# mike-gimelfarb/bboptpy

Hardware: AMD Instinct MI355X
Metric: candidate-evals/sec (higher is better)
Workload: dtype f64; 1 GPU; ActiveCMAES n=128 np=4096 rosenbrock, 256 independent populations per GPU in lockstep; populations_per_gpu=256, n=128, np=4096, objective=rosenbrock

## Files before the change

bboptpy_amd/csrc/bbo_cma.hip:

```cpp
#include "bbo_cma_kernels.hpp"
#include "bbo_sep_kernels.hpp"
#include "bbo_chol_kernels.hpp"
#include "bbo_eig_mw.hpp"

#include <algorithm>
#include <atomic>
#include <cmath>
#include <cstdlib>
#include <limits>

namespace bbo {

namespace {

enum { K_SAMPLE = 0, K_RANK, K_WHITEN, K_GRAM, K_PATHS, K_COV, K_EIGEN, K_POST, K_STOP, K_COUNT };
static const char *const K_NAMES[K_COUNT] = { "bbo:cma_sample_eval", "bbo:cma_rank", "bbo:cma_whiten", "bbo:cma_gram", "bbo:cma_paths", "bbo:cma_cov", "bbo:cma_eigen", "bbo:cma_post", "bbo:cma_history_stop" };

int pick_maxt(int ld)
{
    const int per_wave = ((ld >> 4) + 3) / 4;
    if (per_wave <= 1) return 1;
    if (per_wave <= 2) return 2;
    if (per_wave <= 4) return 4;
    return 8;
// ... 231 lines not shown
        if (params_.adjustlr) c.ccov *= ((n + 2.) / 3.);
    }

    c.rps = 64;
    while (c.rps > 16 && gram_lds_bytes(c.ld, c.rps) > GRAM_LDS_MAX) c.rps >>= 1;
    if (c.ld == 128) {
        int cap = 32;
        if (const char *e = std::getenv("BBO_GRAM_WANT")) cap = std::max(1, std::atoi(e));
        int want = std::max(1, std::min(cap, (512 + P - 1) / P));
        want = std::min(want, (c.lambda_pad + G128_CH - 1) / G128_CH);
        c.rps = ((c.lambda_pad + want - 1) / want + G128_CH - 1) / G128_CH * G128_CH;
    }
    c.splits = (c.lambda_pad + c.rps - 1) / c.rps;
    if (chol) c.splits = 1;
    else if (sep)
        c.splits = std::max(1, std::min(c.mu / 16, (1024 + P - 1) / P));

    const size_t ld = c.ld, ld2 = ld * ld;
    const bool same_shape = dense && keep_bc_ && last_n_ == n && C_.count == P * ld2;
    X_.alloc((size_t) P * c.lambda_pad * ld);
    f_.alloc((size_t) P * c.lambda_pad);
    zn2_.alloc((size_t) P * c.lambda_pad);
    rank_.alloc((size_t) P * c.lambda_pad);
    order_.alloc((size_t) P * c.lambda_pad);
    xmean_.alloc(P * ld);
    xold_.alloc(P * ld);
    pc_.alloc(P * ld);
    ps_.alloc(P * ld);
    D_.alloc(P * ld);
    csep_.alloc(P * ld);
    if (dense) {
        isc_.alloc(P * ld2);
        BDp_.alloc(P * ld2);
        ISp_.alloc(P * ld2);
    }
    if (chol) {
        A_.alloc(P * ld2);
        C_.alloc(P * ld2);
        BDp_.alloc(P * ld2);
        std::vector<double> eyeA(P * ld2, 0.), eyeP(P * ld2, 0.);
        for (int p = 0; p < P; p++)
            for (size_t i = 0; i < (size_t) n; i++) {
                eyeA[p * ld2 + i * ld + i] = 1.;
                eyeP[p * ld2 + bfrag_index(i, i, ld)] = 1.;
            }
        A_.upload(eyeA.data(), P * ld2);
        allow_lds((const void*) chol_factor, 136 * 1024);
        std::vector<int> zero(P, 0);
        chol_repairs_.alloc(P);
        chol_repairs_.upload(zero.data(), P);
        BDp_.upload(eyeP.data(), P * ld2);
    }
    S_.alloc((size_t) P * c.mu_pad);
    gram_part_.alloc((size_t) P * c.splits * (dense ? ld2 : ld));
    mean_part_.alloc((size_t) P * c.splits * ld);
    hist_best_.alloc((size_t) P * c.hlen);
    hist_kth_.alloc((size_t) P * c.hlen);
    weights_.alloc(c.mu);
    weights_.upload(w.data(), c.mu);
    scal_.alloc(P);
    zinject_.release();
    zrecord_.release();
    upload_box(n, c.ld, lower, upper, obj);

    std::vector<double> eye(dense ? P * ld2 : 0, 0.), ones(P * ld, 1.);
    csep_.upload(ones.data(), P * ld);
    if (dense) {
        for (int p = 0; p < P; p++)
            for (int i = 0; i < n; i++) eye[p * ld2 + (size_t) i * ld + i] = 1.;
        if (same_shape) {
            std::vector<double> bm(P * ld2), cm(P * ld2);
            B_.download(bm.data(), P * ld2);
            C_.download(cm.data(), P * ld2);
            for (int p = 0; p < P; p++)
                for (int i = 0; i < n; i++) {
                    bm[p * ld2 + (size_t) i * ld + i] = 1.;
                    cm[p * ld2 + (size_t) i * ld + i] = 1.;
                }
            B_.upload(bm.data(), P * ld2);
            C_.upload(cm.data(), P * ld2);
        } else {
            B_.alloc(P * ld2);
            C_.alloc(P * ld2);
            B_.upload(eye.data(), P * ld2);
            C_.upload(eye.data(), P * ld2);
        }
        isc_.upload(eye.data(), P * ld2);
    }
    D_.upload(ones.data(), P * ld);
    keep_bc_ = dense;
    last_n_ = n;

    std::vector<double> xm(P * ld, 0.);
    for (int p = 0; p < P; p++) std::copy(guess + (size_t) p * n, guess + (size_t) (p + 1) * n,
            xm.begin() + p * ld);
    xmean_.upload(xm.data(), P * ld);

    std::vector<CmaScal> sc(P);
    for (auto &s : sc) {
        std::memset(&s, 0, sizeof(s));
        s.sigma = params_.sigma0;
        s.fbest = -std::numeric_limits<double>::infinity();
        s.fworst = std::numeric_limits<double>::infinity();
        s.hist_head = -1;
        s.basis_ok = same_shape ? 0 : 1;
    }
    scal_.upload(sc.data(), P);
    basis_maybe_stale_ = same_shape;

    if (dense) eig_work_.alloc((size_t) P * 4 * eig_slab((int) ld));

    CmaDev &d = d_;
    d = CmaDev {};
    d.X = X_.p; d.f = f_.p; d.rank = rank_.p; d.order = order_.p;
    d.xmean = xmean_.p; d.xold = xold_.p; d.pc = pc_.p; d.ps = ps_.p;
    d.C = C_.p; d.B = B_.p; d.D = D_.p; d.isc = isc_.p; d.BDp = BDp_.p; d.ISp = ISp_.p;
    d.A = chol ? A_.p : nullptr;
    d.chol_repairs = chol ? chol_repairs_.p : nullptr;
    d.S = S_.p; d.zn2 = zn2_.p; d.csep = csep_.p; d.gram_part = gram_part_.p; d.mean_part = mean_part_.p;
    d.hist_best = hist_best_.p; d.hist_kth = hist_kth_.p; d.eig_work = eig_work_.p;
    d.weights = weights_.p; d.lower = lower_.p; d.upper = upper_.p; d.aux = aux_.p;
    d.zinject = nullptr; d.zrecord = nullptr; d.scal = scal_.p;
    d.stamps = stamps_.p;
    d.mw_fail_host = mw_fail_host_;
    d.mw_fault = mw_fault_from_env();
    mw_release();

    if (obj_.is_program()) {
        prog_.bind(obj_.program, params_.device, n, P);
        std::vector<ProgPlan> plan(P);
        for (int p = 0; p < P; p++)
            plan[p] = ProgPlan { X_.p + (size_t) p * c.lambda_pad * ld, f_.p + (size_t) p * c.lambda_pad, lambda,
                    c.ld };
        prog_.upload_plan(plan);
        std::vector<double> finf((size_t) P * c.lambda_pad, std::numeric_limits<double>::infinity());
        f_.upload(finf.data(), finf.size());
    } else
        prog_.unbind();

    c.honor_stop = 0;
    inited_ = true;
    if (dense) {
        launch_post(2);
        BBO_HIP(hipGetLastError());
        BBO_HIP(hipStreamSynchronize(stream_));
    }
}

void CmaEngine::launch_post(int mode)
{
    const CmaConst &c = c_;
    if (c.ld <= 128) {
        const size_t lds = (size_t) (c.ld * (c.ld + 2) + c.ld) * sizeof(double);
        allow_lds((const void*) cma_post_mfma<1>, 140 * 1024);
        allow_lds((const void*) cma_post_mfma<4>, 140 * 1024);
        if (c.npop < 32)
            hipLaunchKernelGGL(cma_post_mfma<4>, dim3(c.npop, 4), dim3(256), lds, stream_, d_, c_,
                    mode);
        else
            hipLaunchKernelGGL(cma_post_mfma<1>, dim3(c.npop, 1), dim3(256), lds, stream_, d_, c_,
                    mode);
    } else {
        dim3 grid(c.ld / 16, c.ld / 16, c.npop);
        hipLaunchKernelGGL(cma_post, grid, dim3(256), 0, stream_, d_, c_, mode);
    }
}

SampleRoute CmaEngine::sample_route() const
{
    const CmaConst &c = c_;
    SampleRoute r {};
// ... 433 lines not shown
            gens, ldy, scratch);
    BBO_HIP(hipGetLastError());
}

void CmaEngine::generation(bool honor_stop)
{
    if (small_fused_ok()) {
        launch_small(1, honor_stop);
        return;
    }
    small_fused_ = false;
    c_.honor_stop = honor_stop ? 1 : 0;
    launch_sample_eval();
    if (obj_.needs_host()) host_evaluate();
    else if (obj_.is_program()) program_evaluate();
    launch_rank();
    const EigRoute route = eig_route(true, true);
    launch_update(!route.forms_c);
    launch_eigen(route);
    launch_history_stop();
}

void CmaEngine::phase(int which)
{
    BBO_REQUIRE(inited_, "phase before init");
    BBO_HIP(hipSetDevice(params_.device));
    c_.honor_stop = 0;
    d_.mw_fault = mw_fault_from_env();
    switch (which) {
    case BBO_PHASE_SAMPLE_EVALUATE:
        launch_sample_eval();
        if (obj_.needs_host()) host_evaluate();
        else if (obj_.is_program()) program_evaluate();
        break;
    case BBO_PHASE_RANK: launch_rank(); break;
    case BBO_PHASE_UPDATE: launch_update(); break;
    case BBO_PHASE_EIGEN: launch_eigen(eig_route()); break;
    case BBO_PHASE_HISTORY_STOP: launch_history_stop(); break;
    default: throw Error(BBO_ERR_ARG, "unknown CMA phase");
    }
    BBO_HIP(hipStreamSynchronize(stream_));
    if (mw_check_failed() && which == BBO_PHASE_EIGEN) {
        launch_eigen(eig_route());
        BBO_HIP(hipStreamSynchronize(stream_));
    }
    timer_.collect();
    prog_timer_.collect();
}

void CmaEngine::inject_normals(const double *z, int count)
{
    BBO_REQUIRE(inited_, "inject_normals before init");
    rank_wrote_norms_ = false;
    if (!z) {
        d_.zinject = nullptr;
        return;
    }
    const size_t want = (size_t) c_.npop * c_.lambda * c_.n;
    BBO_REQUIRE((size_t) count == want, "inject_normals: count must be populations*lambda*n");
    if (zinject_.count != want) zinject_.alloc(want);
    zinject_.upload(z, want);
    d_.zinject = zinject_.p;
}

void CmaEngine::after_chunk(bool in_run)
{
    if (in_run) return;
    if (mw_check_failed()) {
        launch_eigen(eig_route());
        BBO_HIP(hipStreamSynchronize(stream_));
    }
}

void CmaEngine::inspect(const std::vector<CmaScal> &sc)
{
    bool stale = false;
    for (const auto &s : sc) stale = stale || !s.basis_ok;
    basis_maybe_stale_ = stale;
    mw_check_failed();
    for (const auto &s : sc)
        if (s.eig_mw_fail && !mw_disabled_) {
            mw_disabled_ = true;
            mw_release();
        }
}

int CmaEngine::chunk_limit(int want)
{
    return small_fused_ok() ? std::min(want, 512) : want;
}

void CmaEngine::launch_chunk(int gens)
{
    if (small_fused_ok()) launch_small(gens, true);
    else Engine::launch_chunk(gens);
}

void CmaEngine::solution(int population, double *x_out, int *n_evals, int *converged)
{
    enter_population("solution()", population);
    CmaScal s;
    scal_.download(&s, 1, population);
    std::vector<double> x(c_.ld);
    if (s.it <= 0) xmean_.download(x.data(), c_.ld, (size_t) population * c_.ld);
    else X_.download(x.data(), c_.ld, ((size_t) population * c_.lambda_pad + s.ibw[0]) * c_.ld);
    std::copy(x.begin(), x.begin() + c_.n, x_out);
    *n_evals = s.fev;
    if (s.it <= 0) {
        *converged = c_.variant == 3 ? (c_.tol >= 0. ? 1 : 0) : (0 >= c_.mit) ? 1 : 0;
    } else {
        *converged = s.flag != 0 ? 1 : 0;
    }
}

void CmaEngine::optimize(int n, const double *lower, const double *upper, const double *guess,
// ... 121 lines not shown
            for (int i = 0; i < 48; i++) out[i] = (double) t[i];
        }
        return 48;
    }
    if (k == "best_hist" || k == "kth_hist") {
        if (out && cap >= c.hlen)
            (k == "best_hist" ? hist_best_ : hist_kth_).download(out, c.hlen, (size_t) p * c.hlen);
        return c.hlen;
    }
    CmaScal s;
    scal_.download(&s, 1, p);
    if (k == "sigma") return o.one(s.sigma);
    if (k == "it") return o.one(s.it);
    if (k == "fev") return o.one(s.fev);
    if (k == "flag") return o.one(s.flag);
    if (k == "stop") return o.one(s.stop);
    if (k == "hsig") return o.one(s.hsig);
    if (k == "pslen") return o.one(s.pslen);
    if (k == "fbest") return o.one(s.fbest);
    if (k == "fworst") return o.one(s.fworst);
    if (k == "eigenlastev") return o.one(s.eigenlastev);
    if (k == "eigen_done") return o.one(s.eigen_done);
    if (k == "basis_ok") return o.one(s.basis_ok);
    if (k == "eig_stage") return o.one(s.eig_stage);
    if (k == "eig_mw_fail") return o.one(s.eig_mw_fail);
    if (k == "chol_repairs") {
        if (c.variant != 3) throw Error(BBO_ERR_KEY, "'chol_repairs' belongs to CholeskyCMAES");
        int r = 0;
        chol_repairs_.download(&r, 1, p);
        return o.one(r);
    }
    if (c.variant == 3 && k == "chol_tri") return o.one(chol_tri_ ? 1 : 0);
    if (c.variant == 3 && k == "stol") return o.one(c.stol);
    if (c.variant == 3 && k == "ranked") return o.one(c.ranked);
    if (k == "eig_mw_off") return o.one(mw_disabled_ ? 1 : 0);
    if (k == "eig_split_maxp") return o.one(split_maxp_);
    if (k == "eig_fixed128") return o.one(last_route_.fixed ? 1 : 0);
    if (k == "cov_fused") return o.one(last_route_.forms_c ? 1 : 0);
    if (k == "eig_route") {
        double ids[sizeof(last_route_.step) / sizeof(last_route_.step[0])];
        for (int i = 0; i < last_route_.count; i++) ids[i] = last_route_.step[i].k;
        return o.copy(ids, last_route_.count);
    }
    if (k == "rank_route") return o.one(last_rank_);
    if (k == "sample_route") return o.one(last_sample_.k);
    if (k == "sample_lean") return o.one(last_sample_.full);
    if (k == "update_route") {
        double ids[sizeof(last_update_.step) / sizeof(last_update_.step[0])];
        for (int i = 0; i < last_update_.count; i++) ids[i] = last_update_.step[i].k;
        return o.copy(ids, last_update_.count);
    }
    if (k == "small_fused") return o.one(small_fused_ ? 1 : 0);
    if (k == "splits") return o.one(c.splits);
    if (k == "eig_mw_reserved") return o.one((double) mw_reserved_);
    if (k == "eig_mw_capacity") {
        MwBudget &b = MwBudget::get();
        std::lock_guard<std::mutex> lock(b.m);
        return o.one((double) b.capacity(params_.device));
    }
    if (k == "best_len") return o.one(s.hist_len);
    if (k == "best_buffer") return o.one(s.hist_head);
    if (k == "ibest") return o.one(s.ibw[0]);
    if (k == "ybw") return o.copy(s.ybw, 4);
    if (k == "ibw") {
        const double ids[4] = { (double) s.ibw[0], (double) s.ibw[1], (double) s.ibw[2], (double) s.ibw[3] };
        return o.copy(ids, 4);
    }
    if (k == "n") return o.one(c.n);
    if (k == "lambda") return o.one(c.lambda);
    if (k == "mu") return o.one(c.mu);
    if (k == "mueff") return o.one(c.mueff);
    if (k == "cc") return o.one(c.cc);
    if (k == "cs") return o.one(c.cs);
    if (k == "c1") return o.one(c.c1);
    if (k == "cmu") return o.one(c.cmu);
    if (k == "cneg") return o.one(c.cneg);
    if (k == "alphaold") return o.one(c.alphaold);
    if (k == "cm") return o.one(c.cm);
    if (k == "ccov") return o.one(c.ccov);
    if (k == "damps") return o.one(c.damps);
    if (k == "chi") return o.one(c.chi);
    if (k == "eigenfreq") return o.one(c.eigenfreq);
    if (k == "hlen") return o.one(c.hlen);
    if (k == "ik") return o.one(c.ik);
    if (k == "mit") return o.one(c.mit);
    if (k == "mfev") return o.one(c.mfev);
    if (k == "sigma0") return o.one(c.sigma0);
    throw Error(BBO_ERR_KEY, "unknown state key '" + k + "'");
}

int CmaEngine::set(const std::string &k, int p, const double *in, int count)
{
    enter_population("set()", p);
    rank_wrote_norms_ = false;
    const CmaConst &c = c_;
    const size_t ld = c.ld, n = c.n;
    auto vec_in = [&](DevBuf<double> &b) {
        BBO_REQUIRE(count == (int) n, "set: wrong element count");
        upload_rows(b, p, 1, c.n, c.ld, in);
        return count;
    };
    auto mat_in = [&](DevBuf<double> &b) {
        BBO_REQUIRE(count == (int) (n * n), "set: wrong element count");
        std::vector<double> tmp(ld * ld, 0.);
        for (size_t i = 0; i < n; i++) std::copy(in + i * n, in + (i + 1) * n, tmp.begin() + i * ld);
        b.upload(tmp.data(), ld * ld, p * ld * ld);
        return count;
    };
    if (c.variant == 2 && (k == "B" || k == "C" || k == "D"))
        throw Error(BBO_ERR_KEY, "SepCMAES: set 'csep' (D is its square root)");
    if (c.variant == 3 && (k == "B" || k == "C" || k == "D" || k == "csep"))
        throw Error(BBO_ERR_KEY, "CholeskyCMAES keeps the factor: set 'A'");
    if (k == "A") {
        if (c.variant != 3) throw Error(BBO_ERR_KEY, "'A' belongs to CholeskyCMAES");
        BBO_REQUIRE(count == (int) (n * n), "set: wrong element count");
        std::vector<double> a(ld * ld, 0.), pk(ld * ld, 0.);
        for (size_t i = 0; i < n; i++)
            for (size_t j = 0; j <= i; j++) {
                a[i * ld + j] = in[i * n + j];
                pk[bfrag_index(i, j, ld)] = in[i * n + j];
            }
        A_.upload(a.data(), ld * ld, p * ld * ld);
        BDp_.upload(pk.data(), ld * ld, p * ld * ld);
        return count;
    }
    if (c.variant == 3 && k == "arx") {
        BBO_REQUIRE(count == (int) (c.lambda * n), "set: wrong element count");
        upload_rows(X_, (size_t) p * c.lambda_pad, c.lambda, c.n, c.ld, in);
        return count;
    }
    if (k == "fitness") {
        BBO_REQUIRE(count == c.lambda, "set: wrong element count");
        std::vector<double> f(in, in + c.lambda);
        nan_to_inf(f.data(), c.lambda);
        f_.upload(f.data(), c.lambda, (size_t) p * c.lambda_pad);
        return count;
    }
    if (k == "xmean") return vec_in(xmean_);
    if (k == "xold") return vec_in(xold_);
    if (k == "pc") return vec_in(pc_);
    if (k == "ps") return vec_in(ps_);
    if (k == "csep") {
        BBO_REQUIRE(c.variant == 2, "csep belongs to SepCMAES");
        const int r = vec_in(csep_);
        std::vector<double> dd(ld, 1.);
        for (size_t i = 0; i < n; i++) dd[i] = std::sqrt(in[i]);
        D_.upload(dd.data(), ld, p * ld);
// ... 112 lines not shown
```

bboptpy_amd/csrc/bbo_cma.hpp:

```cpp
#pragma once

#include "bbo_engine.hpp"

namespace bbo {

struct CmaScal {
    double sigma;
    double fbest, fworst;
    double pslen;
    double ybw[4];
    int ibw[4];
    int it, fev;
    int flag;
    int stop;
    int hsig;
    int eigenlastev, eigen_done;
    int hist_head, hist_len;
    int basis_ok;
    int eig_stage;
    int eig_mw_fail;
};

struct CmaConst {
    int n, ld;
    int lambda, lambda_pad;
    int mu, mu_pad;
    int variant;
    int bound, obj;
    int use_zn;
    int lazy_isc;
    int mfev, mit, hlen, ik;
    int honor_stop;
    int splits, rps;
    int npop;
    double mueff, cc, cs, c1, cmu, cneg, alphaold, cm, damps, chi, sigma0, tol, eigenfreq;
    double ccov;
    uint64_t seed;
    int stop_off;
    double ftarget;
    double stol;
    int ranked;
};

enum CmaDbg : int {
    DBG_QL_NO_APPLY      = 1,
    DBG_QL               = 2,
    DBG_DC_NO_MERGES     = 4,
    DBG_DC_NO_LEAVES     = 8,
    DBG_NO_EIGEN_SMALL   = 16,
    DBG_COV_UNFUSED      = 32,
    DBG_NO_SMALL_FUSED   = 64,
    DBG_RANK_COUNT32     = 128,
    DBG_SAMPLE_GUARDED   = 256,
    DBG_GRAM128_LDS      = 512,
    DBG_TRED_L2          = 1024,
    DBG_STAMPS_HALVES    = 2048,
    DBG_RANK_COUNT_NO64  = 4096,
    DBG_DC_ONE_LEVEL     = 8192,
    DBG_DC_TWO_LEVELS    = 16384,
    DBG_DC_LEAF16        = 32768,
    DBG_GRAM_NO_PACING   = 65536,
    DBG_PATHS_LAZY256    = 131072,
    DBG_RANK_BITONIC     = 262144,
    DBG_DC_LEAF_SINGLE   = 524288,
    DBG_SEP_ROWS_LDS     = 1048576,
    DBG_EIG_GENERIC128   = 2097152,
    DBG_EIG_ONE_WG       = 4194304,
    DBG_DC_WG_BARRIERS   = 8388608,
    DBG_TRED_ONE_WG      = 16777216,
    DBG_TOP_PART2        = 33554432,
    DBG_TOP_ONE_KERNEL   = 67108864,
    DBG_WY_PER_WAVE      = 134217728,
    DBG_SAMPLE_4WAVES    = 268435456,
    DBG_TRED_ALL_SPREAD  = 536870912,
    DBG_EIG_IN_KERNEL    = DBG_QL_NO_APPLY | DBG_QL | DBG_DC_NO_MERGES | DBG_DC_NO_LEAVES | DBG_TRED_L2
                           | DBG_STAMPS_HALVES | DBG_DC_ONE_LEVEL | DBG_DC_TWO_LEVELS | DBG_DC_LEAF16
                           | DBG_DC_LEAF_SINGLE | DBG_EIG_ONE_WG | DBG_DC_WG_BARRIERS,
};

struct CmaDev {
    double *X;
    double *f;
    int *rank;
    int *order;
    double *xmean, *xold, *pc, *ps;
    double *C;
    double *B;
    double *D;
    double *isc;
    double *A;
    int *chol_repairs;
    double *BDp;
    double *ISp;
    double *S;
    double *csep;
    double *zn2;
    double *gram_part;
    double *mean_part;
    double *hist_best, *hist_kth;
    double *eig_work;
    const double *weights;
    const double *lower, *upper, *aux;
    const double *zinject;
    double *zrecord;
    CmaScal *scal;
    long long *stamps;
    int dbg;
    int mw_fault;
    int *mw_fail_host;
};

enum EigKernel : int {
    EK_EIGEN_SMALL = 0, EK_EIGEN_128, EK_EIGEN_256, EK_EIGEN, EK_EIGEN_FX128, EK_EIGEN_FX128U,
    EK_EIGEN_R1, EK_EIGEN_R1_FX128, EK_EIGEN_G1, EK_TRED_MW, EK_TRED_TAIL, EK_EIG_HALVES,
    EK_EIGEN_G2, EK_EIG_SECULAR, EK_EIG_LOWNER, EK_EIG_FCOLS, EK_EIGEN_G,
    EK_TRED_MW512, EK_TRED_MW_CHAIN, EK_EIGEN_B4, EK_EIGEN_B,
    EK_EIG_GEMM1, EK_EIG_GEMM, EK_EIG_WY4, EK_EIG_WY4_512, EK_EIG_WY,
    EK_POST, EK_POST_MFMA
};

struct EigRoute {
    struct Step {
        EigKernel k;
        int arg;
    };
    Step step[12];
    int count;
    int timed;
    bool split;
    bool post;
    bool fixed;
    bool forms_c;
    long mw_workgroups;
};

enum SampleKernel : int {
    SK_NONE = -1,
    SK_SEP_16 = 0, SK_SEP_64_512, SK_SEP_64_512_LEAN, SK_SEP_SUM, SK_SEP_SUM4, SK_SEP_64,
    SK_EVAL128, SK_EVAL128_TRI, SK_TILE8, SK_TILE8_TRI,
    SK_EVAL64_1_8, SK_EVAL64_1, SK_EVAL64_2,
    SK_TILE16, SK_EVAL_4, SK_EVAL_8
};

struct SampleRoute {
    SampleKernel k;
    int gx, gy, block;
    size_t lds;
    int rows_per_wg;
    int full;
// ... 48 lines not shown
    }

private:
    static const bbo_params &checked(const bbo_params &p);
    void generation(bool honor_stop) override;
    bool budget_spent(const CmaScal &s) const override { return s.fev >= c_.mfev; }
    void inspect(const std::vector<CmaScal> &sc) override;
    int chunk_limit(int want) override;
    void launch_chunk(int gens) override;
    void after_chunk(bool in_run) override;
    bool small_fused_ok() const;
    void launch_small(int gens, bool honor_stop);
    void launch_sample_eval();
    void launch_post(int mode);
    void launch_rank();
    void launch_update(bool with_cov = true);
    SampleRoute sample_route() const;
    UpdateRoute update_route(bool norms_done, bool with_cov) const;
    EigRoute eig_route(bool spread_ok = true, bool fuse_ok = false) const;
    void launch_eigen(EigRoute r);
    bool nothing_to_guard() const
    {
        return c_.n == c_.ld && !c_.bound && c_.lambda == c_.lambda_pad && !d_.zinject && !d_.zrecord
                && !(d_.dbg & DBG_SAMPLE_GUARDED);
    }
    void launch_history_stop();
    void host_evaluate();
    void program_evaluate();

    CmaConst c_ {};
    CmaDev d_ {};
    bool keep_bc_ = false;
    bool basis_maybe_stale_ = false;
    DevBuf<double> mw_buf_;
    unsigned long long mw_launch_ = 0;
    bool mw_disabled_ = false;
    int mw_xcd_ = next_mw_xcd();
    static int next_mw_xcd();
    long sample_wide_max_tiles_ = 512;
    long sample128_min_rows_ = 256 * 128;
    bool chol_tri_ = true;
    int split_maxp_ = 32;
    EigRoute last_route_ {};
    SampleRoute last_sample_ { SK_NONE };
    UpdateRoute last_update_ {};
    bool small_fused_ = false;
    int last_rank_ = -1;
    bool rank_wrote_norms_ = false;
    int last_n_ = -1;

    DevBuf<double> zn2_, csep_, A_;
    DevBuf<double> X_, f_, xmean_, xold_, pc_, ps_, C_, B_, D_, isc_, BDp_, ISp_, S_,
            gram_part_, mean_part_, hist_best_, hist_kth_, eig_work_, weights_, zinject_, zrecord_;
    DevBuf<int> rank_, order_, chol_repairs_;
    DevBuf<long long> stamps_;
    int *mw_fail_host_ = nullptr;
    long mw_reserved_ = 0;
    bool mw_launched_ = false;
    bool mw_reserve(long workgroups);
    void mw_release();
    bool mw_check_failed();
};

}
```

bboptpy_amd/csrc/bbo_cma_kernels.hpp:

```cpp
#pragma once

#include "bbo_cma.hpp"
#include "bbo_objectives.hpp"
#include "bbo_rng.hpp"
#include "bbo_eig.hpp"
#include "bbo_rank.hpp"

namespace bbo {

typedef double d4_t __attribute__((ext_vector_type(4)));

#define BBO_INF (__builtin_huge_val())

__device__ inline void cma_draw_quad(const CmaDev &d, const CmaConst &c, int p, int row, int q,
        int gen, uint32_t sw, const double2 *tab, double (&z)[4])
{
    const int j0 = cma_quad_col0(q);
    z[0] = z[1] = z[2] = z[3] = 0.;
    if (row < c.lambda && j0 < c.n) {
        if (d.zinject) {
            const double *zi = d.zinject + ((size_t) p * c.lambda + row) * c.n;
#pragma unroll
            for (int i = 0; i < 4; i++)
                if (j0 + 4 * i < c.n) z[i] = zi[j0 + 4 * i];
// ... 471 lines not shown
    __shared__ double ftab[NORMAL_FTABLE_N];
    __shared__ double xms[128];
    normal_table_fill(ntab, tid, 512);
    normal_ftable_fill(ftab, tid, 512);
    if (tid < 128) xms[tid] = d.xmean[(size_t) p * 128 + tid];
    __syncthreads();
    if (full) sample_eval128_body<true, true>(d, c, rows_per_wg, bd, ntab, ftab, xms);
    else sample_eval128_body<false, true>(d, c, rows_per_wg, bd, ntab, ftab, xms);
}

template<int SL>
__device__ __forceinline__ void cma_rank_body(const CmaDev &d, const CmaConst &c)
{
    const int p = blockIdx.y;
    CmaScal *sc = d.scal + p;
    if (pop_frozen(c, sc)) return;
    __shared__ __attribute__((aligned(16))) double tile[RANK_TILE];
    const int tid = threadIdx.x;
    const int cand = blockIdx.x * (256 / SL) + tid / SL, slice = tid % SL;
    const double *f = d.f + (size_t) p * c.lambda_pad;
    const bool live = cand < c.lambda;
    const int cnt = rank_by_counting<SL>(f, c.lambda, cand, slice, tile);
    const bool norms = c.variant == 1 && c.use_zn && sc->basis_ok;
    if (live && slice == 0) {
        const double fi = f[cand];
        d.rank[(size_t) p * c.lambda_pad + cand] = cnt;
        d.order[(size_t) p * c.lambda_pad + cnt] = cand;
        if (cnt == 0) { sc->ibw[0] = cand; sc->ybw[0] = fi; }
        if (cnt == 1) { sc->ibw[1] = cand; sc->ybw[1] = fi; }
        if (cnt == c.lambda - 2) { sc->ibw[2] = cand; sc->ybw[2] = fi; }
        if (cnt == c.lambda - 1) { sc->ibw[3] = cand; sc->ybw[3] = fi; }
        if (norms && cnt >= c.lambda - c.mu)
            d.S[(size_t) p * c.mu_pad + cnt - (c.lambda - c.mu)] =
                    sc->sigma * sc->sigma * d.zn2[(size_t) p * c.lambda_pad + cand];
    }
    if (norms && blockIdx.x == 0)
        for (int wr = c.mu + tid; wr < c.mu_pad; wr += 256) d.S[(size_t) p * c.mu_pad + wr] = 0.;
    if (blockIdx.x == 0 && tid == 0) sc->fev += c.lambda;
}

__global__ __launch_bounds__(256) void cma_rank(CmaDev d, CmaConst c)
{
    cma_rank_body<8>(d, c);
}
__global__ __launch_bounds__(256) void cma_rank32(CmaDev d, CmaConst c)
{
    cma_rank_body<32>(d, c);
}
__global__ __launch_bounds__(256) void cma_rank64(CmaDev d, CmaConst c)
{
    cma_rank_body<64>(d, c);
}

static_assert((int) DBG_RANK_COUNT32 == RANK_DBG_COUNT32 && (int) DBG_RANK_COUNT_NO64 == RANK_DBG_COUNT_NO64
        && (int) DBG_RANK_BITONIC == RANK_DBG_BITONIC, "bbo_rank.hpp reads these bits of CmaDev::dbg");

__global__ __launch_bounds__(1024) void cma_rank_sort(CmaDev d, CmaConst c, int m)
{
    const int p = blockIdx.x;
    CmaScal *sc = d.scal + p;
    if (pop_frozen(c, sc)) return;
    extern __shared__ __attribute__((aligned(16))) double sortbuf[];
    double *keys = sortbuf;
    int *idx = reinterpret_cast<int*>(sortbuf + max(m, 1024));
    const double *f = d.f + (size_t) p * c.lambda_pad;
    int *order = d.order + (size_t) p * c.lambda_pad, *rank = d.rank + (size_t) p * c.lambda_pad;
    if (rank_sort_merges(m, d.dbg)) {
        int *ibuf = reinterpret_cast<int*>(sortbuf + 2 * m);
        if (m == 2048) merge_sort_lds<2>(f, c.lambda, sortbuf, ibuf, order, rank, &keys, &idx);
        else merge_sort_lds<4>(f, c.lambda, sortbuf, ibuf, order, rank, &keys, &idx);
    } else
    bitonic_sort_lds(f, c.lambda, m, keys, idx, order, rank);
    if (c.variant == 1 && c.use_zn && sc->basis_ok) {
        const double s2 = sc->sigma * sc->sigma;
        for (int wr = threadIdx.x; wr < c.mu_pad; wr += blockDim.x)
            d.S[(size_t) p * c.mu_pad + wr] = wr < c.mu
                    ? s2 * d.zn2[(size_t) p * c.lambda_pad + idx[c.lambda - c.mu + wr]] : 0.;
    }
    if (threadIdx.x == 0) {
        const int L = c.lambda;
        sc->ibw[0] = idx[0]; sc->ybw[0] = keys[0];
        sc->ibw[1] = idx[1]; sc->ybw[1] = keys[1];
        sc->ibw[2] = idx[L - 2]; sc->ybw[2] = keys[L - 2];
        sc->ibw[3] = idx[L - 1]; sc->ybw[3] = keys[L - 1];
        sc->fev += L;
    }
}

__device__ __forceinline__ void rank_wave_body(const CmaDev &d, const CmaConst &c, int p, int lane)
{
    CmaScal *sc = d.scal + p;
    if (pop_frozen(c, sc)) return;
    const double *f = d.f + (size_t) p * c.lambda_pad;
    double kf[1] = { lane < c.lambda ? f[lane] : __builtin_huge_val() };
    int ki[1] = { lane < c.lambda ? lane : 0x7fffffff };
    for (int k = 2; k <= 64; k <<= 1)
        for (int j = k >> 1; j > 0; j >>= 1) {
            switch (j) {
            case 1: sort_wave_stage<1, 1>(kf, ki, lane, j, k); break;
            case 2: sort_wave_stage<1, 2>(kf, ki, lane, j, k); break;
            case 4: sort_wave_stage<1, 4>(kf, ki, lane, j, k); break;
            case 8: sort_wave_stage<1, 8>(kf, ki, lane, j, k); break;
            case 16: sort_wave_stage<1, 16>(kf, ki, lane, j, k); break;
            default: sort_wave_stage<1, 32>(kf, ki, lane, j, k); break;
            }
        }
    const int L = c.lambda;
    if (lane < L) {
        d.order[(size_t) p * c.lambda_pad + lane] = ki[0];
        d.rank[(size_t) p * c.lambda_pad + ki[0]] = lane;
        if (lane == 0) { sc->ibw[0] = ki[0]; sc->ybw[0] = kf[0]; }
        if (lane == 1) { sc->ibw[1] = ki[0]; sc->ybw[1] = kf[0]; }
        if (lane == L - 2) { sc->ibw[2] = ki[0]; sc->ybw[2] = kf[0]; }
        if (lane == L - 1) { sc->ibw[3] = ki[0]; sc->ybw[3] = kf[0]; }
    }
    if (lane == 0) sc->fev += L;
}

__global__ __launch_bounds__(256) void cma_rank_wave(CmaDev d, CmaConst c)
{
    const int p = blockIdx.x * 4 + (threadIdx.x >> 6), lane = threadIdx.x & 63;
    if (p >= c.npop) return;
    rank_wave_body(d, c, p, lane);
}

template<int MAXT>
__device__ __forceinline__ void whiten_body(const CmaDev &d, const CmaConst &c, int p, int mt,
        double *lds)
{
    const CmaScal *sc = d.scal + p;
    if (pop_frozen(c, sc)) return;
    const int tid = threadIdx.x, lane = tid & 63, wave = tid >> 6;
    const int ld = c.ld, ldz = ld + 2;
    if (c.use_zn && sc->basis_ok) {
        if (tid < 16) {
            const int wr = mt * 16 + tid;
            if (wr < c.mu_pad)
                d.S[(size_t) p * c.mu_pad + wr] = wr < c.mu
                        ? sc->sigma * sc->sigma * d.zn2[(size_t) p * c.lambda_pad
// ... 230 lines not shown
    if (tg == 0)
        for (int col = tid; col < ld; col += 256) {
            double msum = 0.;
            for (int g = 0; g < rpp; g++) msum += R[g * ld + col];
            d.mean_part[((size_t) p * c.splits + s) * ld + col] = msum;
        }

    const int NT = ld >> 4, LT = NT * (NT + 1) / 2;
    d4_t acc[GRAM_TPW];
    int ti[GRAM_TPW], tj[GRAM_TPW];
#pragma unroll
    for (int t = 0; t < GRAM_TPW; t++) {
        acc[t] = d4_t { 0., 0., 0., 0. };
        const int q = tg * (4 * GRAM_TPW) + wave + 4 * t;
        ti[t] = tj[t] = 0;
        if (q < LT) tri_tile(q, ti[t], tj[t]);
    }
    const int fr = lane & 15, fk = lane >> 4;
    for (int ks = 0; ks < (rlive >> 2); ks++) {
        const int k = 4 * ks + fk;
        const double vk = V[k];
        const double *yk = Y + k * ldy;
#pragma unroll
        for (int t = 0; t < GRAM_TPW; t++) {
            const int q = tg * (4 * GRAM_TPW) + wave + 4 * t;
            if (q < LT) {
                const double a = vk * yk[ti[t] * 16 + fr];
                const double b = yk[tj[t] * 16 + fr];
                acc[t] = __builtin_amdgcn_mfma_f64_16x16x4f64(a, b, acc[t], 0, 0, 0);
            }
        }
    }
    double *G = d.gram_part + ((size_t) p * c.splits + s) * ld * ld;
#pragma unroll
    for (int t = 0; t < GRAM_TPW; t++) {
        const int q = tg * (4 * GRAM_TPW) + wave + 4 * t;
        if (q < LT) {
#pragma unroll
            for (int r = 0; r < 4; r++) {
                const int i = ti[t] * 16 + (lane >> 4) + 4 * r;
                const int j = tj[t] * 16 + (lane & 15);
                G[(size_t) i * ld + j] = acc[t][r];
            }
        }
    }
}

__global__ __launch_bounds__(256) void cma_gram(CmaDev d, CmaConst c, int ldy)
{
    extern __shared__ __attribute__((aligned(16))) double lds[];
    gram_body(d, c, blockIdx.z, blockIdx.x, blockIdx.y, ldy, lds);
}

constexpr int G128_CH = 32;
constexpr int G128_PACE = 2;
constexpr int G128_LDY = 128 + 16;
constexpr int G128_TI[4][9] = { { 5, 5, 5, 6, 6, 6, 7, 7, 7 }, { 2, 2, 2, 3, 3, 3, 4, 4, 4 },
        { 5, 5, 6, 6, 7, 7, 3, 4, 4 }, { 0, 1, 1, 5, 6, 6, 7, 7, 7 } };
constexpr int G128_TJ[4][9] = { { 0, 1, 2, 0, 1, 2, 0, 1, 2 }, { 0, 1, 2, 0, 1, 2, 0, 1, 2 },
        { 3, 4, 3, 4, 3, 4, 3, 3, 4 }, { 0, 0, 1, 5, 5, 6, 5, 6, 7 } };

constexpr bool g128_mean(int wv, int i) { return (wv == 1 && i <= 4) || (wv == 2 && i >= 5); }
constexpr bool g128_needs_a(int wv, int i)
{
    for (int t = 0; t < 9; t++) if (G128_TI[wv][t] == i) return true;
    return false;
}
constexpr bool g128_needs_y(int wv, int i)
{
    for (int t = 0; t < 9; t++) if (G128_TI[wv][t] == i || G128_TJ[wv][t] == i) return true;
    return g128_mean(wv, i);
}

template<int WV>
__device__ inline void gram128_chunk(const double *Yb, const double *Vb, const double *Wb,
        d4_t (&acc)[9], double (&macc)[8], int fr, int fk)
{
#pragma unroll
    for (int ks = 0; ks < G128_CH / 4; ks++) {
        const int k = 4 * ks + fk;
        const double vk = Vb[k];
        const double *yk = Yb + k * G128_LDY + fr;
        double y[8], a[8];
#pragma unroll
        for (int i = 0; i < 8; i++) {
            y[i] = a[i] = 0.;
            if (g128_needs_y(WV, i)) y[i] = yk[i * 16];
            if (g128_needs_a(WV, i)) a[i] = vk * y[i];
        }
        if (WV == 1 || WV == 2) {
            const double wk = Wb[k];
#pragma unroll
            for (int i = 0; i < 8; i++)
                if (g128_mean(WV, i)) macc[i] = fma(wk, y[i], macc[i]);
        }
#pragma unroll
        for (int t = 0; t < 9; t++)
            acc[t] = __builtin_amdgcn_mfma_f64_16x16x4f64(a[G128_TI[WV][t]], y[G128_TJ[WV][t]],
                    acc[t], 0, 0, 0);
    }
}

template<int WV>
__device__ inline void gram128_store(double *G, double *mp, const d4_t (&acc)[9],
        double (&macc)[8], int lane, double isig)
{
    const double isig2 = isig * isig;
// ... 65 lines not shown
        for (int i = 0; i < G128_CH / 8; i++) {
            const int r = r0 + 8 * i;
            const bool in = base + r < c.lambda;
            double2 y01, y23;
            y01.x = (in && in0) ? pf[i][0].x - xo01.x : 0.;
            y01.y = (in && in1) ? pf[i][0].y - xo01.y : 0.;
            y23.x = (in && in2) ? pf[i][1].x - xo23.x : 0.;
            y23.y = (in && in3) ? pf[i][1].y - xo23.y : 0.;
            *reinterpret_cast<double2*>(&Y[buf][r * G128_LDY + c4]) = y01;
            *reinterpret_cast<double2*>(&Y[buf][r * G128_LDY + c4 + 2]) = y23;
        }
        if (tid < G128_CH) {
            V[buf][tid] = pv;
            W[buf][tid] = pw;
        }
    };

    d4_t acc[9];
    double macc[8];
#pragma unroll
    for (int t = 0; t < 9; t++) acc[t] = d4_t { 0., 0., 0., 0. };
#pragma unroll
    for (int i = 0; i < 8; i++) macc[i] = 0.;
    const int fr = lane & 15, fk = lane >> 4;

    fetch(0);
    stash(0, 0);
    __syncthreads();
    for (int ch = 0; ch < nch; ch++) {
        const int buf = ch & 1;
        if (ch + 1 < nch) fetch(ch + 1);
        switch (wave) {
        case 0: gram128_chunk<0>(Y[buf], V[buf], W[buf], acc, macc, fr, fk); break;
        case 1: gram128_chunk<1>(Y[buf], V[buf], W[buf], acc, macc, fr, fk); break;
        case 2: gram128_chunk<2>(Y[buf], V[buf], W[buf], acc, macc, fr, fk); break;
        default: gram128_chunk<3>(Y[buf], V[buf], W[buf], acc, macc, fr, fk); break;
        }
        if (ch + 1 < nch) stash(ch + 1, buf ^ 1);
        __syncthreads();
    }

    double *G = d.gram_part + ((size_t) p * c.splits + s) * 128 * 128;
    double *mp = d.mean_part + ((size_t) p * c.splits + s) * 128;
    switch (wave) {
    case 0: gram128_store<0>(G, mp, acc, macc, lane, isig); break;
    case 1: gram128_store<1>(G, mp, acc, macc, lane, isig); break;
    case 2: gram128_store<2>(G, mp, acc, macc, lane, isig); break;
    default: gram128_store<3>(G, mp, acc, macc, lane, isig); break;
    }
}

template<int WV>
__device__ __forceinline__ void gram128_stream(const CmaDev &d, const CmaConst &c, int p, int s,
        double *coef, int lane)
{
    const CmaScal *sc = d.scal + p;
    const double *Xp = d.X + (size_t) p * c.lambda_pad * 128;
    const double *xold = d.xmean + (size_t) p * 128;
    const int *rank = d.rank + (size_t) p * c.lambda_pad;
    const double isig = 1. / sc->sigma;
    const int row0 = s * c.rps;
    const int nrows = min(c.rps, c.lambda_pad - row0);
    const int nch = (nrows + G128_CH - 1) / G128_CH;
    const int fr = lane & 15, fk = lane >> 4;
    const bool pace = !(d.dbg & DBG_GRAM_NO_PACING);

    double xo[8];
#pragma unroll
    for (int i = 0; i < 8; i++) xo[i] = g128_needs_y(WV, i) ? xold[16 * i + fr] : 0.;
    d4_t acc[9];
    double macc[8];
#pragma unroll
    for (int t = 0; t < 9; t++) acc[t] = d4_t { 0., 0., 0., 0. };
#pragma unroll
    for (int i = 0; i < 8; i++) macc[i] = 0.;

    double ring[4][8];
    const int lane_off = fk * 128 + fr;
    auto load_step = [&](int ch, int ks, int slot) {
        const int blk = min(row0 + ch * G128_CH + 4 * ks, c.lambda_pad - 4);
        const double *src = Xp + (size_t) blk * 128;
#pragma unroll
        for (int i = 0; i < 8; i++)
            if (g128_needs_y(WV, i)) ring[slot][i] = src[lane_off + 16 * i];
    };
    const double cmu1 = c.variant == 1 ? c.cmu + c.cneg * (1. - c.alphaold) : c.cmu;
    const double *Sp = d.S + (size_t) p * c.mu_pad;
    int rk = 0;
    int rk2 = 0;
    double wa = 0., sk = 1., sm = 1.;
    auto coef_link1 = [&](int ch) {
        const int row = row0 + ch * G128_CH + lane;
        const bool ok = lane < G128_CH && ch < nch && row < c.lambda;
        rk = rank[ok ? row : 0];
        if (!ok) rk = -1;
    };
    auto coef_link2 = [&]() {
        rk2 = rk;
        const bool pos = rk2 >= 0 && rk2 < c.mu;
        const int k = min(max(c.lambda - 1 - rk2, 0), c.mu - 1);
        wa = d.weights[pos ? rk2 : k];
        sk = Sp[k];
        sm = Sp[c.mu - 1 - k];
    };
    auto put_coef = [&](int buf) {
        double pv = 0., pw = 0.;
        if (rk2 >= 0 && rk2 < c.mu) {
            pw = wa;
            pv = cmu1 * wa;
        } else if (rk2 >= 0 && c.variant == 1 && rk2 >= c.lambda - c.mu) {
            const double ycoeff = sk / fmax(sm, 1e-8);
            pv = -c.cneg * wa * ycoeff;
        }
        if (lane < G128_CH) {
            coef[buf * 2 * G128_CH + lane] = pv;
            coef[buf * 2 * G128_CH + G128_CH + lane] = pw;
        }
    };
    auto sweep_step = [&](int slot, double vk, double wk) {
        double y[8], a[8];
#pragma unroll
        for (int i = 0; i < 8; i++) {
            y[i] = a[i] = 0.;
            if (g128_needs_y(WV, i)) y[i] = ring[slot][i] - xo[i];
            if (g128_needs_a(WV, i)) a[i] = vk * y[i];
        }
        if (WV == 1 || WV == 2) {
#pragma unroll
            for (int i = 0; i < 8; i++)
                if (g128_mean(WV, i)) macc[i] = fma(wk, y[i], macc[i]);
        }
#pragma unroll
        for (int t = 0; t < 9; t++)
            acc[t] = __builtin_amdgcn_mfma_f64_16x16x4f64(a[G128_TI[WV][t]], y[G128_TJ[WV][t]],
                    acc[t], 0, 0, 0);
    };

    coef_link1(0);
    coef_link2();
    put_coef(0);
    coef_link1(1);
    coef_link2();
    coef_link1(2);
#pragma unroll
    for (int ks = 0; ks < 4; ks++) load_step(0, ks, ks);
    wave_sync();
    for (int ch = 0; ch < nch; ch++) {
        const int buf = ch & 1;
        double vk = coef[buf * 2 * G128_CH + fk], wk = coef[buf * 2 * G128_CH + G128_CH + fk];
#pragma unroll
        for (int ks = 0; ks < 8; ks++) {
            double vn = 0., wn = 0.;
            if (ks < 7) {
                vn = coef[buf * 2 * G128_CH + 4 * (ks + 1) + fk];
                if (WV == 1 || WV == 2) wn = coef[buf * 2 * G128_CH + G128_CH + 4 * (ks + 1) + fk];
            }
            sweep_step(ks & 3, vk, wk);
            vk = vn;
            wk = wn;
            if (ks < 4) load_step(ch, ks + 4, ks & 3);
            else load_step(ch + 1, ks - 4, ks & 3);
            __builtin_amdgcn_sched_barrier(0);
        }
        put_coef(buf ^ 1);
        coef_link2();
        coef_link1(ch + 3);
        wave_sync();
        if (pace && (ch & (G128_PACE - 1)) == G128_PACE - 1) __builtin_amdgcn_s_barrier();
    }
    double *G = d.gram_part + ((size_t) p * c.splits + s) * 128 * 128;
    double *mp = d.mean_part + ((size_t) p * c.splits + s) * 128;
    gram128_store<WV>(G, mp, acc, macc, lane, isig);
}

__global__ __launch_bounds__(256, 2) void cma_gram128s(CmaDev d, CmaConst c)
{
    const int p = blockIdx.y, s = blockIdx.x;
    if (pop_frozen(c, d.scal + p)) return;
    __shared__ double coef[4][2 * 2 * G128_CH];
    const int lane = threadIdx.x & 63, wave = threadIdx.x >> 6;
    switch (wave) {
    case 0: gram128_stream<0>(d, c, p, s, coef[0], lane); break;
    case 1: gram128_stream<1>(d, c, p, s, coef[1], lane); break;
    case 2: gram128_stream<2>(d, c, p, s, coef[2], lane); break;
    default: gram128_stream<3>(d, c, p, s, coef[3], lane); break;
    }
}

template<bool LAZY = false, int T = 256>
__device__ __forceinline__ void paths_body(const CmaDev &d, const CmaConst &c, int p)
{
    CmaScal *sc = d.scal + p;
    if (pop_frozen(c, sc)) return;
    __shared__ double dm[512];
    __shared__ double red[T / 64];
    const int tid = threadIdx.x, ld = c.ld;
    double *xmean = d.xmean + (size_t) p * ld, *xold = d.xold + (size_t) p * ld;
    double *ps = d.ps + (size_t) p * ld, *pc = d.pc + (size_t) p * ld;
    const double sigma = sc->sigma;

    for (int j = tid; j < ld; j += T) {
        double sum = 0.;
        {
            const double *mp = d.mean_part + (size_t) p * c.splits * ld + j;
            int s = 0;
            for (; s + 8 <= c.splits; s += 8) {
                double x[8];
#pragma unroll
                for (int u = 0; u < 8; u++) x[u] = mp[(size_t) (s + u) * ld];
                __builtin_amdgcn_sched_barrier(0);
#pragma unroll
                for (int u = 0; u < 8; u++) sum += x[u];
            }
            for (; s < c.splits; s++) sum += mp[(size_t) s * ld];
        }
        const double xo = xmean[j];
        sum = xo + sigma * sum;
        double xn = 0.;
        if (j < c.n) {
            xn = c.variant == 1 ? xo * (1. - c.cm) + sum * c.cm : sum;
            if (c.bound) xn = fmax(d.lower[j], fmin(xn, d.upper[j]));
        }
        xold[j] = xo;
        xmean[j] = xn;
        dm[j] = xn - xo;
    }
    __syncthreads();

    const double csc = sqrt(c.cs * (2. - c.cs) * c.mueff);
    const double den = c.variant == 1 ? c.cm * sigma : sigma;
    const double *isc = d.isc + (size_t) p * ld * ld;
    double ssq = 0.;
    if (LAZY && sc->basis_ok) {
        constexpr int HN = T / 128;
        constexpr int RS = T / 16, NU = 128 / RS;
        __shared__ double sv[256], cv[256], part[HN - 1][128];
        const double *B = d.B + (size_t) p * ld * ld, *D = d.D + (size_t) p * ld;
        for (int jb = 0; jb < c.n; jb += 128) {
// ... 681 lines not shown
```

Measured before the change: 718.7 million candidate-evals/s.

## Precompute per-row gram coefficients in rank kernel and stream them in gram128

The rank kernel now builds, per population, a table of per-candidate (pv, pw) recombination coefficients using an inverse permutation, and stamps it with the iteration. The gram128 kernel checks the stamp and, when valid, loads coefficients contiguously from the table instead of doing the dependent rank -> weights -> S lookup chain per chunk. This removes serialized gather latency from the inner gram loop at the cost of extra global writes in the rank kernel, added buffer memory, and a stamp check. The table is invalidated when normals are injected or state is set.

```diff
diff --git a/bboptpy_amd/csrc/bbo_cma.hip b/bboptpy_amd/csrc/bbo_cma.hip
--- a/bboptpy_amd/csrc/bbo_cma.hip
+++ b/bboptpy_amd/csrc/bbo_cma.hip
@@ -307,6 +307,9 @@
         BDp_.upload(eyeP.data(), P * ld2);
     }
     S_.alloc((size_t) P * c.mu_pad);
+    const bool coef_table = dense && c.ld == 128;
+    coef_tab_.alloc(coef_table ? (size_t) P * coef_tab_chunks(c.lambda_pad) * 2 * G128_CH : 0);
+    coef_stamp_.alloc(coef_table ? P : 0);
     gram_part_.alloc((size_t) P * c.splits * (dense ? ld2 : ld));
     mean_part_.alloc((size_t) P * c.splits * ld);
     hist_best_.alloc((size_t) P * c.hlen);
@@ -372,6 +375,7 @@
     d.C = C_.p; d.B = B_.p; d.D = D_.p; d.isc = isc_.p; d.BDp = BDp_.p; d.ISp = ISp_.p;
     d.A = chol ? A_.p : nullptr;
     d.chol_repairs = chol ? chol_repairs_.p : nullptr;
+    d.coef_tab = coef_tab_.p; d.coef_stamp = coef_stamp_.p;
     d.S = S_.p; d.zn2 = zn2_.p; d.csep = csep_.p; d.gram_part = gram_part_.p; d.mean_part = mean_part_.p;
     d.hist_best = hist_best_.p; d.hist_kth = hist_kth_.p; d.eig_work = eig_work_.p;
     d.weights = weights_.p; d.lower = lower_.p; d.upper = upper_.p; d.aux = aux_.p;
@@ -911,6 +915,7 @@
 {
     BBO_REQUIRE(inited_, "inject_normals before init");
     rank_wrote_norms_ = false;
+    coef_tab_forget();
     if (!z) {
         d_.zinject = nullptr;
         return;
@@ -920,6 +925,11 @@
     if (zinject_.count != want) zinject_.alloc(want);
     zinject_.upload(z, want);
     d_.zinject = zinject_.p;
+}
+
+void CmaEngine::coef_tab_forget()
+{
+    if (coef_stamp_.p) BBO_HIP(hipMemsetAsync(coef_stamp_.p, 0, coef_stamp_.count * sizeof(int), stream_));
 }
 
 void CmaEngine::after_chunk(bool in_run)
@@ -1147,6 +1157,11 @@
     }
     if (k == "small_fused") return o.one(small_fused_ ? 1 : 0);
     if (k == "splits") return o.one(c.splits);
+    if (k == "gram_coef_stamp") {
+        int stamp = 0;
+        if (coef_stamp_.p) coef_stamp_.download(&stamp, 1, p);
+        return o.one(stamp);
+    }
     if (k == "eig_mw_reserved") return o.one((double) mw_reserved_);
     if (k == "eig_mw_capacity") {
         MwBudget &b = MwBudget::get();
@@ -1188,6 +1203,7 @@
 {
     enter_population("set()", p);
     rank_wrote_norms_ = false;
+    coef_tab_forget();
     const CmaConst &c = c_;
     const size_t ld = c.ld, n = c.n;
     auto vec_in = [&](DevBuf<double> &b) {
diff --git a/bboptpy_amd/csrc/bbo_cma.hpp b/bboptpy_amd/csrc/bbo_cma.hpp
--- a/bboptpy_amd/csrc/bbo_cma.hpp
+++ b/bboptpy_amd/csrc/bbo_cma.hpp
@@ -73,6 +73,7 @@
     DBG_WY_PER_WAVE      = 134217728,
     DBG_SAMPLE_4WAVES    = 268435456,
     DBG_TRED_ALL_SPREAD  = 536870912,
+    DBG_GRAM_LOOKUP      = 1073741824,
     DBG_EIG_IN_KERNEL    = DBG_QL_NO_APPLY | DBG_QL | DBG_DC_NO_MERGES | DBG_DC_NO_LEAVES | DBG_TRED_L2
                            | DBG_STAMPS_HALVES | DBG_DC_ONE_LEVEL | DBG_DC_TWO_LEVELS | DBG_DC_LEAF16
                            | DBG_DC_LEAF_SINGLE | DBG_EIG_ONE_WG | DBG_DC_WG_BARRIERS,
@@ -95,6 +96,8 @@
     double *S;
     double *csep;
     double *zn2;
+    double *coef_tab;
+    int *coef_stamp;
     double *gram_part;
     double *mean_part;
     double *hist_best, *hist_kth;
@@ -249,7 +252,9 @@
     DevBuf<double> zn2_, csep_, A_;
     DevBuf<double> X_, f_, xmean_, xold_, pc_, ps_, C_, B_, D_, isc_, BDp_, ISp_, S_,
             gram_part_, mean_part_, hist_best_, hist_kth_, eig_work_, weights_, zinject_, zrecord_;
-    DevBuf<int> rank_, order_, chol_repairs_;
+    DevBuf<double> coef_tab_;
+    DevBuf<int> rank_, order_, chol_repairs_, coef_stamp_;
+    void coef_tab_forget();
     DevBuf<long long> stamps_;
     int *mw_fail_host_ = nullptr;
     long mw_reserved_ = 0;
diff --git a/bboptpy_amd/csrc/bbo_cma_kernels.hpp b/bboptpy_amd/csrc/bbo_cma_kernels.hpp
--- a/bboptpy_amd/csrc/bbo_cma_kernels.hpp
+++ b/bboptpy_amd/csrc/bbo_cma_kernels.hpp
@@ -547,6 +547,9 @@
     cma_rank_body<64>(d, c);
 }
 
+constexpr int G128_CH = 32;
+__host__ __device__ constexpr int coef_tab_chunks(int lambda_pad) { return (lambda_pad + G128_CH - 1) / G128_CH; }
+
 static_assert((int) DBG_RANK_COUNT32 == RANK_DBG_COUNT32 && (int) DBG_RANK_COUNT_NO64 == RANK_DBG_COUNT_NO64
         && (int) DBG_RANK_BITONIC == RANK_DBG_BITONIC, "bbo_rank.hpp reads these bits of CmaDev::dbg");
 
@@ -580,6 +583,36 @@
         sc->ibw[3] = idx[L - 1]; sc->ybw[3] = keys[L - 1];
         sc->fev += L;
     }
+    if (d.coef_tab && !(d.dbg & DBG_GRAM_LOOKUP) && (c.variant != 1 || (c.use_zn && sc->basis_ok))) {
+        const double cmu1 = c.variant == 1 ? c.cmu + c.cneg * (1. - c.alphaold) : c.cmu;
+        const double s2 = sc->sigma * sc->sigma;
+        const double *zn2 = d.zn2 + (size_t) p * c.lambda_pad;
+        int *inv = reinterpret_cast<int*>(keys);
+        __syncthreads();
+        for (int r = threadIdx.x; r < c.lambda; r += blockDim.x) inv[idx[r]] = r;
+        __syncthreads();
+        const int rows = coef_tab_chunks(c.lambda_pad) * G128_CH;
+        double *tab = d.coef_tab + (size_t) p * rows * 2;
+        for (int row = threadIdx.x; row < rows; row += blockDim.x) {
+            double pv = 0., pw = 0.;
+            if (row < c.lambda) {
+                const int r = inv[row];
+                if (r < c.mu) {
+                    pw = d.weights[r];
+                    pv = cmu1 * pw;
+                } else if (c.variant == 1 && r >= c.lambda - c.mu) {
+                    const int k = c.lambda - 1 - r;
+                    const double sk = s2 * zn2[idx[c.lambda - c.mu + k]], sm = s2 * zn2[row];
+                    const double ycoeff = sk / fmax(sm, 1e-8);
+                    pv = -c.cneg * d.weights[k] * ycoeff;
+                }
+            }
+            double *t = tab + (row / G128_CH) * 2 * G128_CH + row % G128_CH;
+            t[0] = pv;
+            t[G128_CH] = pw;
+        }
+        if (threadIdx.x == 0) d.coef_stamp[p] = sc->it + 1;
+    }
 }
 
 __device__ __forceinline__ void rank_wave_body(const CmaDev &d, const CmaConst &c, int p, int lane)
@@ -916,7 +949,6 @@
     gram_body(d, c, blockIdx.z, blockIdx.x, blockIdx.y, ldy, lds);
 }
 
-constexpr int G128_CH = 32;
 constexpr int G128_PACE = 2;
 constexpr int G128_LDY = 128 + 16;
 constexpr int G128_TI[4][9] = { { 5, 5, 5, 6, 6, 6, 7, 7, 7 }, { 2, 2, 2, 3, 3, 3, 4, 4, 4 },
@@ -1088,7 +1120,7 @@
 
 template<int WV>
 __device__ __forceinline__ void gram128_stream(const CmaDev &d, const CmaConst &c, int p, int s,
-        double *coef, int lane)
+        double *coef, int lane, bool use_tab)
 {
     const CmaScal *sc = d.scal + p;
     const double *Xp = d.X + (size_t) p * c.lambda_pad * 128;
@@ -1123,16 +1155,16 @@
     const double cmu1 = c.variant == 1 ? c.cmu + c.cneg * (1. - c.alphaold) : c.cmu;
     const double *Sp = d.S + (size_t) p * c.mu_pad;
     int rk = 0;
+    bool rk_ok = false;
     int rk2 = 0;
     double wa = 0., sk = 1., sm = 1.;
     auto coef_link1 = [&](int ch) {
         const int row = row0 + ch * G128_CH + lane;
-        const bool ok = lane < G128_CH && ch < nch && row < c.lambda;
-        rk = rank[ok ? row : 0];
-        if (!ok) rk = -1;
+        rk_ok = lane < G128_CH && ch < nch && row < c.lambda;
+        rk = rank[rk_ok ? row : 0];
     };
     auto coef_link2 = [&]() {
-        rk2 = rk;
+        rk2 = rk_ok ? rk : -1;
         const bool pos = rk2 >= 0 && rk2 < c.mu;
         const int k = min(max(c.lambda - 1 - rk2, 0), c.mu - 1);
         wa = d.weights[pos ? rk2 : k];
@@ -1153,6 +1185,14 @@
             coef[buf * 2 * G128_CH + G128_CH + lane] = pw;
         }
     };
+    const double *tabp = d.coef_tab + ((size_t) p * coef_tab_chunks(c.lambda_pad) + row0 / G128_CH) * 2 * G128_CH;
+    unsigned off = 8u * lane;
+    auto tab_load = [&](int ch) {
+        asm volatile("" : "+v"(off));
+        const char *q = reinterpret_cast<const char*>(tabp + min(ch, nch - 1) * 2 * G128_CH);
+        wa = *reinterpret_cast<const double*>(q + off);
+    };
+    auto tab_put = [&](int buf) { coef[buf * 2 * G128_CH + lane] = wa; };
     auto sweep_step = [&](int slot, double vk, double wk) {
         double y[8], a[8];
 #pragma unroll
@@ -1172,12 +1212,19 @@
                     acc[t], 0, 0, 0);
     };
 
-    coef_link1(0);
-    coef_link2();
-    put_coef(0);
-    coef_link1(1);
-    coef_link2();
-    coef_link1(2);
+    const int looks = use_tab ? 0 : G128_CH;
+    if (lane < looks) {
+        coef_link1(0);
+        coef_link2();
+        put_coef(0);
+        coef_link1(1);
+        coef_link2();
+        coef_link1(2);
+    } else if (use_tab) {
+        tab_load(0);
+        tab_put(0);
+        tab_load(1);
+    }
 #pragma unroll
     for (int ks = 0; ks < 4; ks++) load_step(0, ks, ks);
     wave_sync();
@@ -1198,9 +1245,13 @@
             else load_step(ch + 1, ks - 4, ks & 3);
             __builtin_amdgcn_sched_barrier(0);
         }
-        put_coef(buf ^ 1);
-        coef_link2();
-        coef_link1(ch + 3);
+        if (lane < looks) put_coef(buf ^ 1);
+        else if (use_tab) tab_put(buf ^ 1);
+        if (lane < looks) {
+            coef_link2();
+            coef_link1(ch + 3);
+        } else if (use_tab)
+            tab_load(ch + 2);
         wave_sync();
         if (pace && (ch & (G128_PACE - 1)) == G128_PACE - 1) __builtin_amdgcn_s_barrier();
     }
@@ -1215,11 +1266,12 @@
     if (pop_frozen(c, d.scal + p)) return;
     __shared__ double coef[4][2 * 2 * G128_CH];
     const int lane = threadIdx.x & 63, wave = threadIdx.x >> 6;
+    const bool use_tab = d.coef_tab && !(d.dbg & DBG_GRAM_LOOKUP) && d.coef_stamp[p] == d.scal[p].it + 1;
     switch (wave) {
-    case 0: gram128_stream<0>(d, c, p, s, coef[0], lane); break;
-    case 1: gram128_stream<1>(d, c, p, s, coef[1], lane); break;
-    case 2: gram128_stream<2>(d, c, p, s, coef[2], lane); break;
-    default: gram128_stream<3>(d, c, p, s, coef[3], lane); break;
+    case 0: gram128_stream<0>(d, c, p, s, coef[0], lane, use_tab); break;
+    case 1: gram128_stream<1>(d, c, p, s, coef[1], lane, use_tab); break;
+    case 2: gram128_stream<2>(d, c, p, s, coef[2], lane, use_tab); break;
+    default: gram128_stream<3>(d, c, p, s, coef[3], lane, use_tab); break;
     }
 }
 
```

Result: faster. 728.7 million candidate-evals/s, median of 6 (+1.4%).
